# cafferychen777/flashdeconv

Measured on AMD Instinct MI355X. Metric: spots/sec to convergence (1M x 2000 x 30), higher is better.
Workload: dtype f64

## Files before the change

### flashdeconv_amd/_lib.py

```python
import ctypes
import os
import threading

import numpy as np

_HERE = os.path.dirname(os.path.abspath(__file__))
LIB_PATH = os.path.join(_HERE, "libfdx.so")

c_int = ctypes.c_int
c_i32 = ctypes.c_int32
c_i64 = ctypes.c_int64
c_double = ctypes.c_double
c_void_p = ctypes.c_void_p
c_size_t = ctypes.c_size_t
p_double = ctypes.POINTER(ctypes.c_double)
p_i64 = ctypes.POINTER(ctypes.c_int64)
p_i32 = ctypes.POINTER(ctypes.c_int32)


class FdxError(RuntimeError):
    """A libfdx call failed (message from fdx_last_error())."""


class SolveInfo(ctypes.Structure):
# ... 200 lines not shown
    "fdx_comm_init_loopback": (c_int, [c_i32, c_i32, ctypes.POINTER(c_void_p)]),
    "fdx_comm_destroy": (c_int, [c_void_p]),
    "fdx_comm_info": (c_int, [c_void_p, p_i32, p_i32]),
    "fdx_comm_rccl_count": (c_int, [c_void_p, p_i32]),
    "fdx_comm_allreduce_sum_dev": (c_int, [c_void_p, c_void_p, c_i32, c_void_p]),
    "fdx_sharded_solve_dev": (c_int, [c_void_p, c_void_p, c_void_p, c_i64, c_void_p, c_i32, c_double, c_double, c_double, c_i32,
                                      c_void_p, c_void_p, c_i64, ctypes.POINTER(SolveInfo), p_double, p_i32, c_void_p]),
    "fdx_solver_padded_k": (c_i32, [c_i32]),
    "fdx_shard_fit_dev": (c_int, [c_void_p, c_void_p, c_void_p, c_i32, c_i64, c_i32, c_i64, p_double, c_i32, p_i32, p_double, p_double,
                                  ctypes.POINTER(ShardFitParams), c_void_p, c_void_p, p_double, ctypes.POINTER(ShardFitInfo), c_void_p]),
    "fdx_sharded_solve_padded_dev": (c_int, [c_void_p, c_void_p, c_void_p, c_i64, c_void_p, c_i32, c_i32, c_double, c_double, c_double,
                                             c_i32, c_void_p, c_void_p, c_i64, ctypes.POINTER(SolveInfo), p_double, p_i32, c_void_p]),
    "fdx_tile_schedule": (c_int, [p_i32, p_double, c_i32, c_i32, c_i32, c_i32, c_i32, p_i32, p_i32, c_void_p, p_i32, p_double,
                                  c_void_p, c_i64]),
    "fdx_sketch_path": (c_int, [c_i32, c_void_p, c_i64, c_i32, c_i32, c_i32, c_i32, p_i32, p_double, p_i32, p_i32]),
    "fdx_column_sums": (c_int, [c_void_p, c_i32, c_i64, c_i32, p_double]),
    "fdx_log1p_f32": (c_int, [c_void_p, ctypes.c_float, c_i64, c_void_p]),
    "fdx_graph_build_knn": (c_int, [p_double, c_i64, c_i32, c_i32, ctypes.POINTER(c_void_p)]),
    "fdx_graph_build_radius": (c_int, [p_double, c_i64, c_i32, c_double, ctypes.POINTER(c_void_p)]),
    "fdx_nearest_distance": (c_int, [p_double, c_i64, c_i32, p_double]),
    "fdx_graph_export_csr": (c_int, [c_void_p, p_i64, p_i32]),
    "fdx_graph_from_csr": (c_int, [p_i64, p_i64, c_i64, ctypes.POINTER(c_void_p)]),
    "fdx_graph_destroy": (c_int, [c_void_p]),
    "fdx_graph_info": (c_int, [c_void_p, p_i64, p_i64, p_i32]),
    "fdx_graph_knn_ties": (c_int, [c_void_p, p_i64]),
    "fdx_graph_knn_far": (c_int, [c_void_p, ctypes.POINTER(c_i32)]),
    "fdx_kdtree_set_threads": (c_int, [c_i32]),
    "fdx_kdtree_tune": (c_int, [c_i32, c_i64]),
    "fdx_ckdtree_indices_dev": (c_int, [c_void_p, c_i64, c_i32, p_i64, p_i32, c_void_p]),
    "fdx_ckdtree_prebuild": (c_int, [p_double, c_void_p, c_i64, c_i32]),
# ... 135 lines not shown

def ptr_f64(a):
    return a.ctypes.data_as(p_double)


def ptr_i64(a):
    return a.ctypes.data_as(p_i64)


def ptr_i32(a):
    return a.ctypes.data_as(p_i32)


FDX_F32, FDX_F64 = 0, 1
PRE_RAW, PRE_LOG_CPM, PRE_LOG_CPM_SPARSE = 0, 1, 2
PRE_F64_MATH = 0x100


SRC_CODES = {"float32": 0, "float64": 1, "int8": 2, "uint8": 3, "bool": 3, "int16": 4, "uint16": 5, "int32": 6, "uint32": 7,
             "int64": 8, "uint64": 9}
_BIG = 32 << 20


def upload_bytes(dev_ptr, arr):
    if arr.nbytes >= _BIG and arr.nbytes % 4 == 0:
        check(load().fdx_upload_convert_dev(dev_ptr, FDX_F32, arr.ctypes.data_as(c_void_p), SRC_CODES["float32"], arr.nbytes // 4, None, None))
    elif arr.nbytes:
        check(load().fdx_memcpy_h2d(dev_ptr, arr.ctypes.data_as(c_void_p), arr.nbytes, None))


# ... 255 lines not shown
```

### flashdeconv_amd/csrc/fdx_kernels.h

```cpp
#pragma once
#include <cstdlib>
#include <hip/hip_runtime.h>

#include "../../include/fdx.h"
#include "spatial_sums.h"

#include <cstddef>
#include <cstdint>
#include <utility>
#include <initializer_list>

namespace fdx {

constexpr int FDX_MAX_K_FAST = 64;
constexpr int FDX_MAX_K_PAD = 96;
inline int solver_padded_K(int K) {
    if (K <= FDX_MAX_K_FAST || K > FDX_MAX_K_PAD) return K;
    for (int kp : {72, 80, 88, 96})
        if (K <= kp) return kp;
    return K;
}
inline bool sweep_instantiated(int K) { return K >= 1 && (K <= FDX_MAX_K_FAST || K == 72 || K == 80 || K == 88 || K == 96); }

struct BcdSweepArgs {
// ... 41 lines not shown
    const unsigned int* sched_pack = nullptr;
    unsigned long long end_mask = 0ULL;
    int pack_ok = 0;
    const double* gene_w = nullptr;
    const int* gene_bucket = nullptr;
    int scatter_ok = 0;
    const struct SketchPlan* owner = nullptr;
};
inline bool sketch_scatter_fits(int G, int d) {
    return d < 65535 && (((size_t)G + 256 + 7) & ~(size_t)7) * 10 + ((size_t)d + 64) * 8 <= 150 * 1024;
}
int launch_sketch_rows(const void* Y, int dtype, long long ldy, const int* row_map, long long n, int G, int d, int mode,
                       const SketchPlanDev& plan, double* Ys, long long ldys, double* row_sumsq, hipStream_t st);
bool fused_sketch_contract_ok(int dtype, long long ldy, const void* Y, int G, int d, int K, int mode, const SketchPlanDev& plan,
                              hipStream_t st = nullptr);
struct TileF64Math {
    bool prev;
    explicit TileF64Math(bool on);
    ~TileF64Math();
};
bool tile_sketch_ok(int dtype, long long ldy, const void* Y, int G, int d, int K, int mode, const SketchPlanDev& plan, hipStream_t st);
int launch_tile_sketch(const void* Y, int dtype, long long ldy, const int* row_map, long long n, int G, int d, int mode,
                       const SketchPlanDev& plan, const double* Xs, int K, double* H, long long ldh, double* row_sumsq,
                       hipStream_t st);
int launch_sketch_contract(const void* Y, int dtype, long long ldy, const int* row_map, long long n, int G, int d, int mode,
                           const SketchPlanDev& plan, const double* Xs, int K, double* H, long long ldh, double* row_sumsq,
                           hipStream_t st);
int column_sums_parts(long long n);
int launch_column_sums(const void* Y, int dtype, long long ldy, long long n, int G, double* partials, double* out,
                       hipStream_t st);
// ... 94 lines not shown
```

### flashdeconv_amd/csrc/fit.cpp

```cpp
#include "fdx_env.h"
#include <algorithm>
#include <cstdio>
#include <cmath>
#include <cstdlib>
#include <memory>
#include <vector>

#include "fdx_graph.h"
#include "fdx_internal.h"
#include "fdx_kernels.h"
#include "graph_build.h"
#include "prepare.h"
#include "sketch_plan.h"
#include "solver.h"
#include "x_cache.h"

using namespace fdx;

namespace {

int build_csc_from_tables(const int32_t* bucket, const double* weight, int G, int d, std::vector<long long>* col_ptr,
                          std::vector<int>* gene_idx, std::vector<double>* w) {
    col_ptr->assign((size_t)d + 1, 0);
    for (int g = 0; g < G; ++g) {
// ... 295 lines not shown
namespace {

std::unique_ptr<fdx_fit_carry> adopt_carry(const fdx_fit_params* prm) {
    return std::unique_ptr<fdx_fit_carry>(prm ? static_cast<fdx_fit_carry*>(prm->carry) : nullptr);
}

int fit_impl(const YSource& ysrc, int64_t n, int32_t G, const double* X, int32_t K, const int32_t* bucket,
             const double* weight_y, const double* weight_x, const double* coords_dev, int32_t dim,
             const fdx_fit_params* prm_in, std::unique_ptr<fdx_fit_carry> carry_in, fdx_graph** graph_inout, double* beta_out_dev,
             double* prop_out_dev, double* objectives_out, double* rel_changes_out, fdx_fit_info* info, void* stream) {
    FDX_REQUIRE(info != nullptr && prm_in != nullptr && graph_inout != nullptr, "fdx_fit_dev: null argument");
    fdx_fit_params prm_local = *prm_in;
    prm_local.mode_y &= 0xff;
    const fdx_fit_params* prm = &prm_local;
    TileF64Math f64_math((prm_in->mode_y & FDX_PRE_F64_MATH) != 0);
    std::memset(info, 0, sizeof(*info));
    const int32_t y_dtype = ysrc.row_dtype();
    FDX_REQUIRE(y_dtype == FDX_F32 || y_dtype == FDX_F64, "fdx_fit_dev: Y dtype must be FDX_F32 or FDX_F64");
    FDX_REQUIRE(n > 0 && G > 0 && K > 0, "fdx_fit_dev: empty problem");
    FDX_REQUIRE(n < 0x7fffff00LL, "fdx_fit_dev: n too large for one device");
    FDX_REQUIRE(ysrc.csr || ysrc.ldy >= G, "fdx_fit_dev: ldy < G");
    FDX_REQUIRE((ysrc.dense || ysrc.csr) && X && bucket && weight_y && weight_x, "fdx_fit_dev: null array");
    const int d = prm->sketch_dim;
    FDX_REQUIRE(d > 0, "fdx_fit_dev: sketch_dim must be positive");
    FDX_REQUIRE(prm->max_iter >= 0, "fdx_fit_dev: max_iter must be non-negative");
    hipStream_t st = (hipStream_t)stream;
    PoolStream pool_stream(st);
    Event t_begin(true), t_graph(true), eS0(true), eS1(true), t_solved(true), t_end(true);
    FDX_TRY(t_begin.record(st));
    trace_host("fit", "entry");
// ... 294 lines not shown
```

### flashdeconv_amd/csrc/prepare.cpp

```cpp
#include "prepare.h"

#include <algorithm>
#include <cstring>
#include <vector>

#include "fdx_env.h"
#include "fdx_kernels.h"
#include "solver.h"

namespace fdx {

int YTables::build(const YSource& y, int G, int d, int K, const int32_t* bucket, const double* weight_y, hipStream_t xs,
                   const char* who) {
    if (!y.csr) return sketch_plan_cached(bucket, weight_y, G, d, xs, &plan);
    csr_fused = csr_contract_ok(d, K, (y.csr->G + 31) / 32);
    return sel.build(y.gene_idx, G, y.csr->G, bucket, weight_y, d, csr_fused, xs, who);
}

namespace {
XCache<XSideBufs>& x_side_cache() {
    static XCache<XSideBufs>* const c = new XCache<XSideBufs>(4);
    return *c;
}
}
// ... 113 lines not shown
        Event sketched;
        FDX_TRY(sketched.record(st));
        FDX_TRY(sketched.wait_on(ys));
    }
    FDX_TRY(launch_sum_partials(row_sq, n, sum_dev, 1, 1, ys));
    if (yty_host) FDX_HIP(hipMemcpyAsync(yty_host, sum_dev, sizeof(double), hipMemcpyDeviceToHost, ys));
    if (done && ys != st) FDX_TRY(done->record(ys));
    return 0;
}

int prepare_queue(PrepareJob* job, const void* Y_dev, int y_dtype, long long n, int G, long long ldy, const int* row_map_dev,
                  const double* X, int K, const int* bucket, const double* weight_y, const double* weight_x, int d, int mode_y_in,
                  int mode_x, double* H_out_dev, long long ldh, double* XtX_host, hipStream_t st, const double* X_dev) {
    const int32_t mode_y = mode_y_in & 0xff;
    TileF64Math f64_math((mode_y_in & FDX_PRE_F64_MATH) != 0);
    FDX_REQUIRE(y_dtype == FDX_F32 || y_dtype == FDX_F64, "fdx_prepare_dev: Y dtype must be FDX_F32 or FDX_F64");
    FDX_REQUIRE(n >= 0 && G > 0 && K > 0 && d > 0, "fdx_prepare_dev: bad shape");
    FDX_REQUIRE(X && bucket && weight_y && weight_x && H_out_dev, "fdx_prepare_dev: null array");
    FDX_REQUIRE(ldh >= n && ldy >= G, "fdx_prepare_dev: leading dimension too small");
    YSource ysrc;
    ysrc.dense = Y_dev;
    ysrc.dtype = y_dtype;
    ysrc.ldy = ldy;
    hipStream_t side = fdx::env("FDX_NO_SIDE_STREAM") ? nullptr : library_side_stream();
    if (side == st) side = nullptr;
    job->side = side;
    const hipStream_t xs = side ? side : st;
    {
        PoolStream pool_xs(xs);
        FDX_TRY(job->y.build(ysrc, G, d, K, bucket, weight_y, xs, "fdx_prepare_dev"));
// ... 14 lines not shown
```

### flashdeconv_amd/csrc/tile_kernels.cpp

```cpp
#include "fdx_env.h"
#include <algorithm>
#include <cmath>
#include <cstdlib>
#include <memory>
#include <mutex>

#include "fdx_internal.h"
#include "fdx_kernels.h"
#include "sketch_plan.h"
#include "tile_device.h"
#include "tile_plan.h"
#include "tile_variant.h"

namespace fdx {

struct TilePlanDevice {
    TilePlanHost h;
    DevBuf w, off, len, ent_base, slot_bucket;
    int RS = 0;
    int WB = 0;
    size_t lds = 0;
};

const double* log_table_dev(hipStream_t st) {
    static std::mutex mu;
    static double* tabs[64] = {};
    int dev = 0;
    if (hipGetDevice(&dev) != hipSuccess || dev < 0 || dev >= 64) return nullptr;
    std::lock_guard<std::mutex> lock(mu);
    if (!tabs[dev]) {
        std::vector<double> t((size_t)LOG_TAB_N);
        for (int i = 0; i < LOG_TAB_N; ++i) {
            const unsigned bits = (unsigned)(LOG_TAB_BASE + i) << LOG_TAB_SHIFT;
            float c;
            std::memcpy(&c, &bits, 4);
            t[(size_t)i] = (double)(-logl((long double)c) + (long double)LOG_TAB_EXP_SHIFT * 0.693147180559945309417232121458176568L);
// ... 1 lines not shown
        double* p = nullptr;
        if (hipMalloc(&p, t.size() * sizeof(double)) != hipSuccess) return nullptr;
        if (hipMemcpyAsync(p, t.data(), t.size() * sizeof(double), hipMemcpyHostToDevice, st) != hipSuccess ||
            hipStreamSynchronize(st) != hipSuccess) {
            (void)hipFree(p);
            return nullptr;
        }
        tabs[dev] = p;
    }
    return tabs[dev];
}

static thread_local bool t_f64_math = false;
TileF64Math::TileF64Math(bool on) : prev(t_f64_math) { t_f64_math = on; }
TileF64Math::~TileF64Math() { t_f64_math = prev; }

static int tile_logv() {
    if (t_f64_math) return 0;
    const char* e = fdx::env("FDX_TILE_LOGV");
    return e ? atoi(e) : 2;
}

static bool tile_cfg(int dtype, int mode, int K, int d, int logv, TileVariant* out) {
    if ((dtype != FDX_F32 && dtype != FDX_F64) || K < 1 || K > 64 || d < 1) return false;
    if (mode != FDX_PRE_RAW && mode != FDX_PRE_LOG_CPM && mode != FDX_PRE_LOG_CPM_SPARSE) return false;
    const bool raw = mode == FDX_PRE_RAW;
    TileVariant v = raw ? TileVariant{12, 4, 11} : TileVariant{16, 0, 8};
    v.TT = (K + 15) / 16;
    if (K > 32 || d > 4 * v.NWC * v.JW) {
        v = raw ? TileVariant{12, 4, 22, 4, true} : TileVariant{8, 0, 32, 4, true};
// ... 62 lines not shown
        wg_tab.assign((size_t)t.h.NBLK * per, 0.0);
        for (int g = 0; g < sp.G; ++g)
            if (sp.host_bucket[(size_t)g] >= 0) wg_tab[(size_t)(g / t.h.GB) * per + g % t.h.GB] = sp.host_w[(size_t)g];
        for (size_t i = 0; i < t.h.off.size(); ++i)
            if (t.h.gene[i] < 0) t.h.off[i] = (unsigned short)t.h.GB;
    }
    if ((t.WB ? up(t.w, wg_tab.data(), wg_tab.size() * 8) : up(t.w, t.h.w.data(), t.h.w.size() * 8)) ||
        up(t.off, t.h.off.data(), t.h.off.size() * 2) || up(t.len, len_pad.data(), len_pad.size()) || up(t.ent_base, t.h.ent_base.data(), t.h.ent_base.size() * 4) ||
        up(t.slot_bucket, t.h.slot_bucket.data(), t.h.slot_bucket.size() * 4))
        return nullptr;
    if (hipStreamSynchronize(st) != hipSuccess) return nullptr;
    sp.tile[key] = std::move(best);
    return sp.tile[key].get();
}

__global__ void tile_xa_kernel(const double* __restrict__ Xs, const int* __restrict__ slot_bucket, int K, int d, int n_groups,
                               int TT, double* __restrict__ XA) {
    const int i = blockIdx.x * blockDim.x + threadIdx.x;
    if (i >= n_groups * TT * 64) return;
    const int lane = i & 63, t = (i >> 6) % TT, wj = (i >> 6) / TT;
    const int b = slot_bucket[wj * 4 + (lane >> 4)];
    const int type = t * 16 + (lane & 15);
    XA[i] = (b >= 0 && type < K) ? Xs[(size_t)type * d + b] : 0.0;
}

bool tile_sketch_ok(int dtype, long long ldy, const void* Y, int G, int d, int K, int mode, const SketchPlanDev& plan,
                    hipStream_t st) {
    if (!plan.owner) return false;
    TileVariant v;
    if (G <= 0 || !tile_cfg(dtype, mode, K, d, tile_logv(), &v)) return false;
    const int sz = dtype == FDX_F32 ? 4 : 8;
    if ((K > 32 || d > 512) && fdx::env("FDX_NO_TILE_WIDE")) return false;
    if (((size_t)G * sz) % 16 != 0 || ((size_t)ldy * sz) % 16 != 0 || (reinterpret_cast<uintptr_t>(Y) & 15) != 0) return false;
    return tile_plan_for(*plan.owner, dtype, mode, v, st) != nullptr;
}

int launch_tile_sketch(const void* Y, int dtype, long long ldy, const int* row_map, long long n, int G, int d, int mode,
                       const SketchPlanDev& plan, const double* Xs, int K, double* H, long long ldh, double* row_sumsq,
                       hipStream_t st) {
    if (n <= 0) return 0;
    TileVariant v;
    const TilePlanDevice* t = plan.owner && tile_cfg(dtype, mode, K, d, tile_logv(), &v) ? tile_plan_for(*plan.owner, dtype, mode, v, st) : nullptr;
    if (!t) return fail(FDX_ERR_INVALID, "tile sketch: no schedule for this shape");
    const void* kern = dtype == FDX_F32 ? tile_kernel<float>(mode, v) : tile_kernel<double>(mode, v);
    if (!kern) {
        char msg[128];
        std::snprintf(msg, sizeof msg, "tile sketch: no kernel for dtype %d mode %d, waves %d + %d x %d, TT %d, AVL2 %d, LOGV %d, WG %d",
                      dtype, mode, v.NWC, v.NWL, v.JW, v.TT, (int)v.avl2, v.logv, (int)v.wg);
        return fail(FDX_ERR_INVALID, msg);
    }
    TileArgs a{};
    a.ldy = ldy; a.n = n; a.ldh = ldh; a.G = G; a.d = d; a.K = K;
    a.NE = t->h.NE; a.GB = t->h.GB; a.NBLK = t->h.NBLK; a.RS = t->RS; a.jw_used = t->h.jw_used; a.WB = t->WB;
    const double* w_tab = t->w.as<double>();
    const unsigned short* off_tab = t->off.as<unsigned short>();
    const unsigned char* len_tab = t->len.as<unsigned char>();
    const int* ent_base = t->ent_base.as<int>();
    const int* slot_bucket = t->slot_bucket.as<int>();
// ... 73 lines not shown
    std::copy(h.slot_bucket.begin(), h.slot_bucket.end(), slot_bucket_out);
    std::copy(h.len.begin(), h.len.end(), len_out);
    std::copy(h.ent_base.begin(), h.ent_base.end(), ent_base_out);
    std::copy(h.w.begin(), h.w.end(), w_out);
    std::copy(h.off.begin(), h.off.end(), off_out);
    return 0;
}

extern "C" int fdx_sketch_path(int32_t y_dtype, const void* Y_dev, int64_t ldy, int32_t G, int32_t d, int32_t K, int32_t mode_y_in,
                               const int32_t* bucket, const double* weight_y, int32_t* path_out,
                               int32_t* dims_out ) {
    using namespace fdx;
    FDX_REQUIRE(bucket && weight_y && path_out, "fdx_sketch_path: null argument");
    FDX_REQUIRE(G > 0 && K > 0 && d > 0 && ldy >= G, "fdx_sketch_path: bad shape");
    const int32_t mode_y = mode_y_in & 0xff;
    if (dims_out) std::fill(dims_out, dims_out + 6, 0);
    hipStream_t st = nullptr;
    PoolStream pool_stream(st);
    std::shared_ptr<SketchPlan> plan;
    FDX_TRY(sketch_plan_cached(bucket, weight_y, G, d, st, &plan));
    *path_out = 0;
    if (!fused_sketch_contract_ok(y_dtype, ldy, Y_dev, G, d, K, mode_y, plan->dev(), st)) return 0;
    TileVariant v;
    const TilePlanDevice* t = tile_cfg(y_dtype, mode_y, K, d, tile_logv(), &v) ? tile_plan_for(*plan, y_dtype, mode_y, v, st) : nullptr;
    FDX_REQUIRE(t != nullptr, "fdx_sketch_path: the one-kernel form was accepted without a schedule");
    *path_out = v.wide ? 2 : 1;
    if (dims_out) {
        dims_out[0] = v.NWC; dims_out[1] = v.NWL; dims_out[2] = v.JW; dims_out[3] = v.TT;
        dims_out[4] = t->h.GB; dims_out[5] = t->h.NBLK;
    }
    return 0;
}
```

### flashdeconv_amd/csrc/tile_plan.cpp

```cpp
#include "tile_plan.h"

#include <algorithm>
#include <numeric>

namespace fdx {

bool build_tile_plan(const int* gene_bucket, const double* gene_w, int G, int d, int NW, int JW, int GB, TilePlanHost* out) {
    if (G <= 0 || d <= 0 || NW <= 0 || JW <= 0 || GB <= 0 || GB > 65536) return false;
    const int n_groups = NW * JW;
    if (d > 4 * n_groups) return false;
    const int NBLK = (G + GB - 1) / GB;
    TilePlanHost& p = *out;
    p = TilePlanHost();
    p.G = G; p.d = d; p.NW = NW; p.JW = JW; p.GB = GB; p.NBLK = NBLK;

    std::vector<std::vector<int>> genes((size_t)d);
    for (int g = 0; g < G; ++g) {
        const int b = gene_bucket[g];
        if (b < 0) continue;
        if (b >= d) return false;
        genes[(size_t)b].push_back(g);
    }
    std::vector<int> cnt((size_t)d * NBLK, 0);
    for (int b = 0; b < d; ++b)
// ... 95 lines not shown
            p.off.push_back(0);
            p.gene.push_back(-1);
        }
        p.steps += wave_steps;
        p.max_wave_steps = std::max(p.max_wave_steps, wave_steps);
        for (int j = 0; j < JW; ++j)
            for (int q = 0; q < 4; ++q) {
                const int b = groups[(size_t)of_wave[(size_t)w][(size_t)j]].b[q];
                if (b >= 0 && taken[(size_t)j * 4 + q] != (int)genes[(size_t)b].size()) return false;
            }
    }
    p.NE = (int)p.w.size();
    return true;
}

}
```

### flashdeconv_amd/csrc/tile_plan.h

```cpp
#pragma once
#include <vector>

namespace fdx {

struct TilePlanHost {
    int G = 0, d = 0, NW = 0, JW = 0, GB = 0, NBLK = 0;
    int NE = 0;
    int steps = 0;
    int max_wave_steps = 0;
    int jw_used = 0;
    std::vector<int> slot_bucket;
    std::vector<unsigned char> len;
    std::vector<int> ent_base;
    std::vector<double> w;
    std::vector<unsigned short> off;
    std::vector<int> gene;
};

bool build_tile_plan(const int* gene_bucket, const double* gene_w, int G, int d, int NW, int JW, int GB, TilePlanHost* out);


}
```

### flashdeconv_amd/csrc/tile_variant.h

```cpp
#pragma once
#include <cstddef>

namespace fdx {

constexpr int TILE_ROW_PAD = 16;

struct TileArgs {
    long long ldy, n, ldh;
    int G, d, K;
    int NE, GB, NBLK, RS, jw_used;
    int WB;
};

constexpr int JW_PAD(int jw) { return (jw + 7) & ~7; }

constexpr bool tile_red_pair(int NWC, bool AVL2) { return NWC > 8 || AVL2; }
constexpr int tile_red_th(int TT) { return TT > 2 ? 2 : TT; }
constexpr size_t tile_red_bytes(int NWC, bool AVL2, int TT) {
    return (size_t)(tile_red_pair(NWC, AVL2) ? NWC / 2 : NWC) * (tile_red_th(TT) * 4 * 64 + 64) * 8;
}

struct TileVariant {
    int NWC, NWL, JW, TT;
    bool wide, avl2;
    int logv;
    bool wg;
};

template <typename T> const void* tile_kernel(int mode, const TileVariant& v);

}
```

### include/fdx.h

```cpp
#ifndef FDX_H
#define FDX_H

#include <stddef.h>
#include <stdint.h>

#ifdef __cplusplus
extern "C" {
#endif

#define FDX_OK 0
#define FDX_ERR_INVALID (-1)
#define FDX_ERR_HIP (-2)
#define FDX_ERR_UNSUPPORTED (-3)
#define FDX_ERR_INTERNAL (-4)

#define FDX_F32 0
#define FDX_F64 1

#define FDX_PRE_RAW 0
#define FDX_PRE_LOG_CPM 1
#define FDX_PRE_LOG_CPM_SPARSE 2
#define FDX_PRE_F64_MATH 0x100

int fdx_version(void);
int fdx_env_reload(void);
const char* fdx_env_switch(int32_t i, const char** what_out);
const char* fdx_last_error(void);
int fdx_device_count(int* count);
int fdx_set_device(int device);
int fdx_device_name(char* buf, int buflen);

int fdx_malloc(void** dev_ptr, size_t bytes);
int fdx_free(void* dev_ptr);
int fdx_trim(void);
int fdx_x_cache_stats(int64_t out[4]);
int fdx_memcpy_h2d(void* dev_dst, const void* host_src, size_t bytes, void* stream);
int fdx_memcpy_d2h(void* host_dst, const void* dev_src, size_t bytes, void* stream);
// ... 10 lines not shown
#define FDX_SRC_U32 7
#define FDX_SRC_I64 8
#define FDX_SRC_U64 9
int fdx_upload_convert_dev(void* dst_dev, int32_t dst_dtype, const void* src_host, int32_t src_code, int64_t count,
                           double* max_abs_out, void* stream);
int fdx_download_dev(void* dst_host, const void* src_dev, size_t bytes, void* stream);
int fdx_pinned_copy_rate(size_t bytes, int32_t to_device, double* gbps_out);

int fdx_sketch(const void* Y, int32_t dtype, int64_t n, int32_t G, const int64_t* col_ptr, const int32_t* gene_idx,
               const double* weight, int32_t d, int32_t mode, double* Ys_out);
int fdx_tile_schedule(const int32_t* gene_bucket, const double* gene_w, int32_t G, int32_t d, int32_t NW, int32_t JW,
                      int32_t GB, int32_t* dims_out, int32_t* slot_bucket_out, uint8_t* len_out, int32_t* ent_base_out,
                      double* w_out, uint16_t* off_out, int64_t cap_entries);
int fdx_sketch_path(int32_t y_dtype, const void* Y_dev, int64_t ldy, int32_t G, int32_t d, int32_t K, int32_t mode_y,
                    const int32_t* bucket, const double* weight_y, int32_t* path_out, int32_t* dims_out);
int fdx_log1p_f32(const float* y, float scale, int64_t n, float* out);
int fdx_column_sums(const void* Y, int32_t dtype, int64_t n, int32_t G, double* sums_out);

int fdx_column_sums_dev(const void* Y_dev, int32_t dtype, int64_t n, int32_t G, int64_t ldy, double* sums_out_host,
                        void* stream);

int fdx_gene_moments_dev(const void* Y_dev, int32_t dtype, int64_t n, int32_t G, int64_t ldy, double* mean_out_host,
                         double* var_out_host, void* stream);
int fdx_gather_columns_dev(const void* Y_dev, int32_t dtype, int64_t n, int32_t G, int64_t ldy, const int32_t* idx_host,
                           int32_t G_sel, void* out_dev, void* stream);

int fdx_leverage_scores(const double* X, int32_t K, int32_t G, double regularization, double* lev_out);
typedef struct fdx_leverage_job fdx_leverage_job;
int fdx_leverage_begin(const double* X, int32_t K, int32_t G, double regularization, fdx_leverage_job** job);
int fdx_leverage_end(fdx_leverage_job* job, double* lev_out);
// ... 343 lines not shown
```

Baseline: 284.6 million.

## Add 64-spot tiled sketch kernel with per-wave gene batch schedule

Adds a new fused sketch-and-contract kernel that processes 64 spots per tile. Gene rows are double-buffered into LDS, per-wave batched gene schedules scatter weighted values into register accumulators, and the sketch is contracted against X with f64 MFMA after permlane swaps. A host-side planner builds the 64-spot batch schedule, and mode flags let callers force the 16- or 64-spot path. The aim is more reuse per loaded row and less scheduling overhead, at the cost of a much more complex kernel with high register pressure and possible occupancy limits.

```diff
diff --git a/flashdeconv_amd/_lib.py b/flashdeconv_amd/_lib.py
--- a/flashdeconv_amd/_lib.py
+++ b/flashdeconv_amd/_lib.py
@@ -238,6 +238,7 @@
     "fdx_tile_schedule": (c_int, [p_i32, p_double, c_i32, c_i32, c_i32, c_i32, c_i32, p_i32, p_i32, c_void_p, p_i32, p_double,
                                   c_void_p, c_i64]),
     "fdx_sketch_path": (c_int, [c_i32, c_void_p, c_i64, c_i32, c_i32, c_i32, c_i32, p_i32, p_double, p_i32, p_i32]),
+    "fdx_sketch_tile_spots": (c_int, [c_i32, c_void_p, c_i64, c_i32, c_i32, c_i32, c_i32, p_i32, p_double, c_i64, p_i32]),
     "fdx_column_sums": (c_int, [c_void_p, c_i32, c_i64, c_i32, p_double]),
     "fdx_log1p_f32": (c_int, [c_void_p, ctypes.c_float, c_i64, c_void_p]),
     "fdx_graph_build_knn": (c_int, [p_double, c_i64, c_i32, c_i32, ctypes.POINTER(c_void_p)]),
@@ -403,6 +404,7 @@
 
 FDX_F32, FDX_F64 = 0, 1
 PRE_RAW, PRE_LOG_CPM, PRE_LOG_CPM_SPARSE = 0, 1, 2
+PRE_TILE16, PRE_TILE64 = 0x200, 0x400
 PRE_F64_MATH = 0x100
 
 
diff --git a/flashdeconv_amd/csrc/fdx_kernels.h b/flashdeconv_amd/csrc/fdx_kernels.h
--- a/flashdeconv_amd/csrc/fdx_kernels.h
+++ b/flashdeconv_amd/csrc/fdx_kernels.h
@@ -79,6 +79,11 @@
                        const SketchPlanDev& plan, double* Ys, long long ldys, double* row_sumsq, hipStream_t st);
 bool fused_sketch_contract_ok(int dtype, long long ldy, const void* Y, int G, int d, int K, int mode, const SketchPlanDev& plan,
                               hipStream_t st = nullptr);
+struct TileSpotsForce {
+    int prev;
+    explicit TileSpotsForce(int mode_y_in);
+    ~TileSpotsForce();
+};
 struct TileF64Math {
     bool prev;
     explicit TileF64Math(bool on);
diff --git a/flashdeconv_amd/csrc/fit.cpp b/flashdeconv_amd/csrc/fit.cpp
--- a/flashdeconv_amd/csrc/fit.cpp
+++ b/flashdeconv_amd/csrc/fit.cpp
@@ -333,6 +333,7 @@
     prm_local.mode_y &= 0xff;
     const fdx_fit_params* prm = &prm_local;
     TileF64Math f64_math((prm_in->mode_y & FDX_PRE_F64_MATH) != 0);
+    TileSpotsForce tile_spots_force(prm_in->mode_y);
     std::memset(info, 0, sizeof(*info));
     const int32_t y_dtype = ysrc.row_dtype();
     FDX_REQUIRE(y_dtype == FDX_F32 || y_dtype == FDX_F64, "fdx_fit_dev: Y dtype must be FDX_F32 or FDX_F64");
diff --git a/flashdeconv_amd/csrc/hosttest/plan64_asan.cpp b/flashdeconv_amd/csrc/hosttest/plan64_asan.cpp
--- /dev/null
+++ b/flashdeconv_amd/csrc/hosttest/plan64_asan.cpp
@@ -0,0 +1,76 @@
+#include <cstdio>
+#include <cstring>
+#include <random>
+#include <vector>
+
+#include "../tile_plan.h"
+
+using namespace fdx;
+
+static int check_tile64(int G, int d, int GB16, int elem_bytes, unsigned seed) {
+    const int NW = T64_NW, JW = T64_JW, GB = T64_ROW_BYTES / elem_bytes;
+    std::mt19937 rng(seed);
+    std::vector<int> bucket((size_t)G);
+    std::vector<double> w((size_t)G);
+    for (int g = 0; g < G; ++g) {
+        bucket[(size_t)g] = (rng() % 41 == 0) ? -1 : (int)(rng() % (unsigned)d);
+        w[(size_t)g] = (rng() & 1) ? 1.0 + (rng() % 100) * 0.01 : -1.0 - (rng() % 100) * 0.01;
+    }
+    TilePlanHost p16;
+    if (!build_tile_plan(bucket.data(), w.data(), G, d, NW, JW, GB16, &p16)) return 1;
+    Tile64PlanHost p;
+    if (!build_tile64_plan(bucket.data(), w.data(), G, d, p16.slot_bucket.data(), NW, JW, GB, elem_bytes, &p)) return 2;
+    if (p.NBLK != (G + GB - 1) / GB || (int)p.words.size() != (p.n_batches + 2) * T64_BATCH_WORDS ||
+        (int)p.gene.size() != (p.n_batches + 2) * T64_U || (int)p.batch_base.size() != NW * (3 * p.NBLK + 1))
+        return 3;
+    std::vector<int> seen((size_t)G, 0), last((size_t)d, -1);
+    int at = 0;
+    for (int wv = 0; wv < NW; ++wv) {
+        const int* bb = p.batch_base.data() + (size_t)wv * (3 * p.NBLK + 1);
+        if (bb[0] != at) return 4;
+        for (int c = 0; c < p.NBLK; ++c)
+            for (int seg = 0; seg < 3; ++seg)
+                for (int b = bb[3 * c + seg]; b < bb[3 * c + seg + 1]; ++b, ++at) {
+                    if (b != at) return 5;
+                    const int* e = p.words.data() + (size_t)b * T64_BATCH_WORDS;
+                    for (int u = 0; u < T64_U; ++u) {
+                        const unsigned m = (unsigned)e[2 * T64_U + u];
+                        const int idx = (int)((m >> 16) & 0xff), off = (int)(m & 0xffffu);
+                        double wt;
+                        const unsigned long long bits = ((unsigned long long)(unsigned)e[2 * u + 1] << 32) | (unsigned)e[2 * u];
+                        std::memcpy(&wt, &bits, 8);
+                        if ((int)(m >> 24) != seg || idx >= 16 || seg * 16 + idx >= JW * 4 || off + elem_bytes > T64_ROW_BYTES) return 6;
+                        const int g = p.gene[(size_t)b * T64_U + u];
+                        if (g < 0) {
+                            if (wt != 0.0 || off != 0) return 7;
+                            continue;
+                        }
+                        const int own = p16.slot_bucket[(size_t)wv * JW * 4 + seg * 16 + idx];
+                        if (g / GB != c || own != bucket[(size_t)g] || wt != w[(size_t)g] || off != (g % GB) * elem_bytes) return 8;
+                        if (g <= last[(size_t)own]) return 9;
+                        last[(size_t)own] = g;
+                        ++seen[(size_t)g];
+                    }
+                }
+        if (bb[3 * p.NBLK] != at) return 10;
+    }
+    if (at != p.n_batches) return 11;
+    for (int g = 0; g < G; ++g)
+        if (seen[(size_t)g] != (bucket[(size_t)g] >= 0 ? 1 : 0)) return 12;
+    for (size_t i = (size_t)p.n_batches * T64_U; i < p.gene.size(); ++i)
+        if (p.gene[i] != -1) return 13;
+    return 0;
+}
+
+int main() {
+    int bad = 0;
+    const int shapes[][4] = {{2000, 512, 1024, 4}, {2000, 528, 1024, 4}, {1500, 256, 384, 8}, {600, 64, 768, 4}, {64, 512, 256, 4},
+                             {256, 64, 256, 4}, {4, 8, 256, 4}, {2, 1, 128, 8}};
+    for (const auto& s : shapes)
+        for (unsigned seed = 1; seed <= 3; ++seed) {
+            const int rc = check_tile64(s[0], s[1], s[2], s[3], seed);
+            if (rc) { std::printf("tile64 plan G=%d d=%d GB16=%d bytes=%d seed=%u: error %d\n", s[0], s[1], s[2], s[3], seed, rc); ++bad; }
+        }
+    std::printf(bad ? "FAILED\n" : "64-spot schedule builder: ok under the sanitizers\n");
+    return bad ? 1 : 0;
+}
diff --git a/flashdeconv_amd/csrc/prepare.cpp b/flashdeconv_amd/csrc/prepare.cpp
--- a/flashdeconv_amd/csrc/prepare.cpp
+++ b/flashdeconv_amd/csrc/prepare.cpp
@@ -151,6 +151,7 @@
                   int mode_x, double* H_out_dev, long long ldh, double* XtX_host, hipStream_t st, const double* X_dev) {
     const int32_t mode_y = mode_y_in & 0xff;
     TileF64Math f64_math((mode_y_in & FDX_PRE_F64_MATH) != 0);
+    TileSpotsForce tile_spots_force(mode_y_in);
     FDX_REQUIRE(y_dtype == FDX_F32 || y_dtype == FDX_F64, "fdx_prepare_dev: Y dtype must be FDX_F32 or FDX_F64");
     FDX_REQUIRE(n >= 0 && G > 0 && K > 0 && d > 0, "fdx_prepare_dev: bad shape");
     FDX_REQUIRE(X && bucket && weight_y && weight_x && H_out_dev, "fdx_prepare_dev: null array");
diff --git a/flashdeconv_amd/csrc/tile64_inst.cpp b/flashdeconv_amd/csrc/tile64_inst.cpp
--- /dev/null
+++ b/flashdeconv_amd/csrc/tile64_inst.cpp
@@ -0,0 +1,17 @@
+#include "tile64_sketch_kernel.h"
+
+#ifndef FDX_TILE_F64
+#error "compile with -DFDX_TILE_F64=<0|1>"
+#endif
+
+namespace fdx {
+
+using TileT = std::conditional<FDX_TILE_F64, double, float>::type;
+
+template <> const void* tile64_kernel<TileT>(int TT) {
+    if (TT == 1) return (const void*)tile64_sketch_kernel<TileT, 1>;
+    if (TT == 2) return (const void*)tile64_sketch_kernel<TileT, 2>;
+    return nullptr;
+}
+
+}
diff --git a/flashdeconv_amd/csrc/tile64_sketch_kernel.h b/flashdeconv_amd/csrc/tile64_sketch_kernel.h
--- /dev/null
+++ b/flashdeconv_amd/csrc/tile64_sketch_kernel.h
@@ -0,0 +1,229 @@
+#pragma once
+#include <type_traits>
+
+#include "tile_sketch_kernel.h"
+
+namespace fdx {
+
+typedef double t64_d16 __attribute__((ext_vector_type(16)));
+
+template <int I0, int I1, typename F> __device__ __forceinline__ void t64_static_for(F&& f) {
+    if constexpr (I0 < I1) {
+        f(std::integral_constant<int, I0>{});
+        t64_static_for<I0 + 1, I1>(f);
+    }
+}
+
+__device__ __forceinline__ void t64_swap32(double& a, double& b) {
+    const auto lo = __builtin_amdgcn_permlane32_swap((unsigned)__double2loint(a), (unsigned)__double2loint(b), false, false);
+    const auto hi = __builtin_amdgcn_permlane32_swap((unsigned)__double2hiint(a), (unsigned)__double2hiint(b), false, false);
+    a = __hiloint2double((int)hi[0], (int)lo[0]);
+    b = __hiloint2double((int)hi[1], (int)lo[1]);
+}
+__device__ __forceinline__ void t64_swap16(double& a, double& b) {
+    const auto lo = __builtin_amdgcn_permlane16_swap((unsigned)__double2loint(a), (unsigned)__double2loint(b), false, false);
+    const auto hi = __builtin_amdgcn_permlane16_swap((unsigned)__double2hiint(a), (unsigned)__double2hiint(b), false, false);
+    a = __hiloint2double((int)hi[0], (int)lo[0]);
+    b = __hiloint2double((int)hi[1], (int)lo[1]);
+}
+
+template <typename T, int TT>
+__global__ __launch_bounds__(T64_NW * 64, T64_NW / 4) void tile64_sketch_kernel(
+    const TileArgs a, const T* __restrict__ Yp, const int* __restrict__ row_map, const double* __restrict__ Xs,
+    double* __restrict__ H, double* __restrict__ row_sumsq, const int* __restrict__ ent, const int* __restrict__ batch_base,
+    const int* __restrict__ slot_bucket) {
+    extern __shared__ __attribute__((aligned(16))) unsigned char smem[];
+    static_assert(TT == 1 || TT == 2, "narrow form: one or two type tiles");
+    constexpr int NW = T64_NW, JW = T64_JW, U = T64_U, W = T64_BATCH_WORDS;
+    constexpr int RPL = (T64_ROWS + NW - 1) / NW;
+    constexpr int NR = NW / 2;
+    constexpr int TS = 4 * 64;
+    static_assert(tile64_red_bytes() == (size_t)2 * NR * (TS + 64) * 8, "the reduction area overlays a stage buffer");
+    const int tid = threadIdx.x, lane = tid & 63;
+    const int wave = __builtin_amdgcn_readfirstlane(tid >> 6);
+    const int r = lane & 15, q = lane >> 4;
+    const int stage_bytes = T64_ROWS * a.RS;
+    const long long n_tiles = (a.n + T64_ROWS - 1) / T64_ROWS;
+    long long tile = blockIdx.x;
+    if (tile >= n_tiles) return;
+
+    auto load_rows = [&](long long t, const T* (&rp)[RPL]) {
+#pragma unroll
+        for (int k = 0; k < RPL; ++k) {
+            const int rr = wave + NW * k;
+            rp[k] = nullptr;
+            if (rr >= T64_ROWS || t >= n_tiles) continue;
+            const long long sp = t * T64_ROWS + rr;
+            if (sp < a.n) {
+                const long long row = row_map ? (long long)row_map[sp] : sp;
+                rp[k] = Yp + (size_t)row * (size_t)a.ldy;
+            }
+        }
+    };
+    auto issue_stage = [&](const T* const (&rp)[RPL], int c, int buf) {
+        const int gene0 = c * a.GB;
+        const int bytes = (min(a.GB, a.G - gene0)) * (int)sizeof(T);
+        unsigned char* base = smem + (size_t)buf * stage_bytes;
+#pragma unroll
+        for (int k = 0; k < RPL; ++k) {
+            if (!rp[k]) continue;
+            const unsigned char* src = reinterpret_cast<const unsigned char*>(rp[k] + gene0) + lane * 16;
+            if (lane * 16 < bytes) dma16(src, base + (wave + NW * k) * a.RS);
+        }
+    };
+    const T* rowp[RPL];
+    const T* rown[RPL];
+    load_rows(tile, rowp);
+    issue_stage(rowp, 0, 0);
+
+    const int* bb = batch_base + wave * (3 * a.NBLK + 1);
+    int buf = 0;
+    for (; tile < n_tiles; tile += gridDim.x) {
+        const bool has_next = tile + gridDim.x < n_tiles;
+        load_rows(tile + gridDim.x, rown);
+        t64_d16 A = (t64_d16)(0.0), B = (t64_d16)(0.0);
+        t64_d16 C = (t64_d16)(0.0);
+        for (int c = 0; c < a.NBLK; ++c) {
+            __builtin_amdgcn_s_waitcnt(0x0f70);
+            lds_barrier();
+            if (c + 1 < a.NBLK) issue_stage(rowp, c + 1, buf ^ 1);
+            else if (has_next) issue_stage(rown, 0, buf ^ 1);
+            const unsigned rowb = (unsigned)buf * (unsigned)stage_bytes + (unsigned)lane * (unsigned)a.RS;
+            int b = bb[3 * c];
+            const int b1 = bb[3 * c + 1], b2 = bb[3 * c + 2], b3 = bb[3 * c + 3];
+            auto fetch = [&](int (&e)[W], int bi) {
+#pragma unroll
+                for (int i = 0; i < W; ++i) e[i] = ent[(size_t)bi * W + i];
+            };
+            auto read = [&](T (&y)[U], const int (&e)[W]) {
+#pragma unroll
+                for (int u = 0; u < U; ++u) y[u] = *reinterpret_cast<const T*>(smem + rowb + ((unsigned)e[2 * U + u] & 0xffffu));
+            };
+            int e[W], en[W];
+            T y[U];
+            fetch(e, b);
+            fetch(en, b + 1);
+            read(y, e);
+            auto run = [&](auto& V, int bend) __attribute__((always_inline)) {
+                while (b < bend) {
+                    double yd[U];
+#pragma unroll
+                    for (int u = 0; u < U; ++u) yd[u] = (double)y[u];
+                    __builtin_amdgcn_sched_barrier(0);
+                    read(y, en);
+                    int e2[W];
+                    fetch(e2, b + 2);
+                    __builtin_amdgcn_sched_barrier(0);
+#pragma unroll
+                    for (int u = 0; u < U; ++u) {
+                        const int i = (e[2 * U + u] >> 16) & 15;
+                        V[i] = fma(__hiloint2double(e[2 * u + 1], e[2 * u]), yd[u], V[i]);
+                    }
+                    ++b;
+#pragma unroll
+                    for (int i = 0; i < W; ++i) {
+                        e[i] = en[i];
+                        en[i] = e2[i];
+                    }
+                }
+            };
+            run(A, b1);
+            run(B, b2);
+            run(C, b3);
+            buf ^= 1;
+        }
+#pragma unroll
+        for (int k = 0; k < RPL; ++k) rowp[k] = rown[k];
+
+        double av[JW];
+        auto load_av = [&](int t) {
+            int sb0 = wave * JW * 4;
+            asm volatile("" : "+s"(sb0));
+#pragma unroll
+            for (int j = 0; j < JW; ++j) {
+                const int c0 = slot_bucket[sb0 + j * 4], c1 = slot_bucket[sb0 + j * 4 + 1], c2 = slot_bucket[sb0 + j * 4 + 2],
+                          c3 = slot_bucket[sb0 + j * 4 + 3];
+                const int b = q == 0 ? c0 : q == 1 ? c1 : q == 2 ? c2 : c3;
+                const int type = t * 16 + r;
+                const bool ok = b >= 0 && type < a.K;
+                const double v = Xs[(size_t)(ok ? type : 0) * a.d + (ok ? b : 0)];
+                av[j] = ok ? v : 0.0;
+            }
+        };
+        load_av(0);
+        auto get = [&](auto jc, auto qc) -> double {
+            constexpr int J = decltype(jc)::value, QQ = decltype(qc)::value;
+            if constexpr (J < 4) return A[J * 4 + QQ];
+            else if constexpr (J < 8) return B[(J - 4) * 4 + QQ];
+            else return C[(J - 8) * 4 + QQ];
+        };
+        auto set = [&](auto jc, auto qc, double v) {
+            constexpr int J = decltype(jc)::value, QQ = decltype(qc)::value;
+            if constexpr (J < 4) A[J * 4 + QQ] = v;
+            else if constexpr (J < 8) B[(J - 4) * 4 + QQ] = v;
+            else C[(J - 8) * 4 + QQ] = v;
+        };
+        using I0 = std::integral_constant<int, 0>;
+        using I1 = std::integral_constant<int, 1>;
+        using I2 = std::integral_constant<int, 2>;
+        using I3 = std::integral_constant<int, 3>;
+        t64_static_for<0, JW>([&](auto jc) {
+            double r0 = get(jc, I0{}), r1 = get(jc, I1{}), r2 = get(jc, I2{}), r3 = get(jc, I3{});
+            t64_swap32(r0, r2);
+            t64_swap32(r1, r3);
+            t64_swap16(r0, r1);
+            t64_swap16(r2, r3);
+            set(jc, I0{}, r0);
+            set(jc, I1{}, r1);
+            set(jc, I2{}, r2);
+            set(jc, I3{}, r3);
+        });
+        double* red_base = reinterpret_cast<double*>(smem + (size_t)(buf ^ 1) * stage_bytes);
+        lds_barrier();
+        t64_static_for<0, 4 * TT>([&](auto rc) {
+            constexpr int TI = decltype(rc)::value / 4, S = decltype(rc)::value % 4;
+            if (TI > 0 && S == 0) load_av(TI);
+            using SC = std::integral_constant<int, S>;
+            double* red = red_base + (size_t)(decltype(rc)::value & 1) * NR * (TS + 64);
+            double* red_sq = red + (size_t)NR * TS;
+            double4_t accm = double4_t{0.0, 0.0, 0.0, 0.0};
+            double sq = 0.0;
+            t64_static_for<0, JW>([&](auto jc) {
+                constexpr int J = decltype(jc)::value;
+                const double bv = get(jc, SC{});
+                accm = __builtin_amdgcn_mfma_f64_16x16x4f64(av[J], bv, accm, 0, 0, 0);
+                if (TI == 0) sq = fma(bv, bv, sq);
+            });
+            if (wave >= NR) {
+#pragma unroll
+                for (int rr = 0; rr < 4; ++rr) red[(size_t)(wave - NR) * TS + rr * 64 + lane] = accm[rr];
+                if (TI == 0) red_sq[(wave - NR) * 64 + lane] = sq;
+            }
+            lds_barrier();
+            if (wave < NR) {
+#pragma unroll
+                for (int rr = 0; rr < 4; ++rr) red[(size_t)wave * TS + rr * 64 + lane] += accm[rr];
+                if (TI == 0) red_sq[wave * 64 + lane] += sq;
+            }
+            lds_barrier();
+            const long long s0 = tile * T64_ROWS + S * TILE_ROWS;
+            if (tid < TS) {
+                double sum = 0.0;
+#pragma unroll
+                for (int v = 0; v < NR; ++v) sum += red[(size_t)v * TS + tid];
+                const int type = TI * 16 + (lane >> 4) + 4 * (tid >> 6);
+                const long long sp = s0 + (lane & 15);
+                if (type < a.K && sp < a.n) H[(size_t)type * a.ldh + sp] = sum;
+            }
+            if (TI == 0 && row_sumsq && tid < TILE_ROWS && s0 + tid < a.n) {
+                double sum = 0.0;
+                for (int v = 0; v < NR; ++v)
+#pragma unroll
+                    for (int qq = 0; qq < 4; ++qq) sum += red_sq[v * 64 + qq * 16 + tid];
+                row_sumsq[s0 + tid] = sum;
+            }
+        });
+    }
+}
+
+}
diff --git a/flashdeconv_amd/csrc/tile_kernels.cpp b/flashdeconv_amd/csrc/tile_kernels.cpp
--- a/flashdeconv_amd/csrc/tile_kernels.cpp
+++ b/flashdeconv_amd/csrc/tile_kernels.cpp
@@ -14,12 +14,19 @@
 
 namespace fdx {
 
+struct Tile64PlanDevice {
+    Tile64PlanHost h;
+    DevBuf words, batch_base;
+};
+
 struct TilePlanDevice {
     TilePlanHost h;
     DevBuf w, off, len, ent_base, slot_bucket;
     int RS = 0;
     int WB = 0;
     size_t lds = 0;
+    mutable std::unique_ptr<Tile64PlanDevice> t64;
+    mutable bool t64_tried = false;
 };
 
 const double* log_table_dev(hipStream_t st) {
@@ -51,6 +58,12 @@
 static thread_local bool t_f64_math = false;
 TileF64Math::TileF64Math(bool on) : prev(t_f64_math) { t_f64_math = on; }
 TileF64Math::~TileF64Math() { t_f64_math = prev; }
+
+static thread_local int t_tile_spots = 0;
+TileSpotsForce::TileSpotsForce(int mode_y_in) : prev(t_tile_spots) {
+    t_tile_spots = (mode_y_in & FDX_PRE_TILE64) ? 64 : (mode_y_in & FDX_PRE_TILE16) ? 16 : 0;
+}
+TileSpotsForce::~TileSpotsForce() { t_tile_spots = prev; }
 
 static int tile_logv() {
     if (t_f64_math) return 0;
@@ -143,6 +156,55 @@
     return sp.tile[key].get();
 }
 
+static int tile_spots(int mode, const TileVariant& v) {
+    const bool can = mode == FDX_PRE_RAW && !v.wide && v.NWC == T64_NW && v.JW == T64_JW;
+    return can && t_tile_spots == 64 ? 64 : 16;
+}
+
+static const Tile64PlanDevice* tile64_plan_for(const SketchPlan& sp, int dtype, const TilePlanDevice& t, hipStream_t st) {
+    std::lock_guard<std::mutex> lock(sp.tile_mu);
+    if (t.t64_tried) return t.t64.get();
+    t.t64_tried = true;
+    const int sz = dtype == FDX_F32 ? 4 : 8;
+    auto p = std::make_unique<Tile64PlanDevice>();
+    if (!build_tile64_plan(sp.host_bucket.data(), sp.host_w.data(), sp.G, sp.d, t.h.slot_bucket.data(), T64_NW, T64_JW,
+                           T64_ROW_BYTES / sz, sz, &p->h))
+        return nullptr;
+    if (p->words.alloc(p->h.words.size() * 4) || copy_h2d(p->words.p, p->h.words.data(), p->h.words.size() * 4, st) ||
+        p->batch_base.alloc(p->h.batch_base.size() * 4) ||
+        copy_h2d(p->batch_base.p, p->h.batch_base.data(), p->h.batch_base.size() * 4, st))
+        return nullptr;
+    if (hipStreamSynchronize(st) != hipSuccess) return nullptr;
+    if (fdx::env("FDX_DEBUG"))
+        std::fprintf(stderr, "[fdx] tile64 plan: G=%d d=%d GB=%d blocks=%d batches=%d (%d entries for %d genes)\n", sp.G, sp.d, p->h.GB,
+                     p->h.NBLK, p->h.n_batches, p->h.n_batches * T64_U, sp.G);
+    t.t64 = std::move(p);
+    return t.t64.get();
+}
+
+static int launch_tile64(const void* Y, int dtype, long long ldy, const int* row_map, long long n, int G, int d, const SketchPlan& sp,
+                         const TilePlanDevice& t, const TileVariant& v, const double* Xs, int K, double* H, long long ldh,
+                         double* row_sumsq, hipStream_t st) {
+    const Tile64PlanDevice* p = tile64_plan_for(sp, dtype, t, st);
+    if (!p) return fail(FDX_ERR_INVALID, "tile sketch: no 64-spot schedule for this shape");
+    const void* kern = dtype == FDX_F32 ? tile64_kernel<float>(v.TT) : tile64_kernel<double>(v.TT);
+    if (!kern) return fail(FDX_ERR_INVALID, "tile sketch: no 64-spot kernel for this number of type tiles");
+    TileArgs a{};
+    a.ldy = ldy; a.n = n; a.ldh = ldh; a.G = G; a.d = d; a.K = K;
+    a.GB = p->h.GB; a.NBLK = p->h.NBLK; a.RS = T64_ROW_BYTES + TILE_ROW_PAD;
+    const int* ent = p->words.as<int>();
+    const int* batch_base = p->batch_base.as<int>();
+    const int* slot_bucket = t.slot_bucket.as<int>();
+    const long long n_tiles = (n + T64_ROWS - 1) / T64_ROWS;
+    const int grid = (int)std::min<long long>(n_tiles, 256);
+    const size_t lds = tile64_lds_bytes();
+    FDX_HIP(hipFuncSetAttribute(kern, hipFuncAttributeMaxDynamicSharedMemorySize, (int)lds));
+    void* args[] = {(void*)&a, (void*)&Y, (void*)&row_map, (void*)&Xs, (void*)&H, (void*)&row_sumsq, (void*)&ent, (void*)&batch_base,
+                    (void*)&slot_bucket};
+    FDX_HIP(hipLaunchKernel(kern, dim3(grid), dim3(T64_NW * 64), args, lds, st));
+    return 0;
+}
+
 __global__ void tile_xa_kernel(const double* __restrict__ Xs, const int* __restrict__ slot_bucket, int K, int d, int n_groups,
                                int TT, double* __restrict__ XA) {
     const int i = blockIdx.x * blockDim.x + threadIdx.x;
@@ -171,6 +233,7 @@
     TileVariant v;
     const TilePlanDevice* t = plan.owner && tile_cfg(dtype, mode, K, d, tile_logv(), &v) ? tile_plan_for(*plan.owner, dtype, mode, v, st) : nullptr;
     if (!t) return fail(FDX_ERR_INVALID, "tile sketch: no schedule for this shape");
+    if (tile_spots(mode, v) == 64) return launch_tile64(Y, dtype, ldy, row_map, n, G, d, *plan.owner, *t, v, Xs, K, H, ldh, row_sumsq, st);
     const void* kern = dtype == FDX_F32 ? tile_kernel<float>(mode, v) : tile_kernel<double>(mode, v);
     if (!kern) {
         char msg[128];
@@ -274,6 +337,7 @@
     FDX_REQUIRE(bucket && weight_y && path_out, "fdx_sketch_path: null argument");
     FDX_REQUIRE(G > 0 && K > 0 && d > 0 && ldy >= G, "fdx_sketch_path: bad shape");
     const int32_t mode_y = mode_y_in & 0xff;
+    TileSpotsForce tile_spots_force(mode_y_in);
     if (dims_out) std::fill(dims_out, dims_out + 6, 0);
     hipStream_t st = nullptr;
     PoolStream pool_stream(st);
@@ -288,6 +352,25 @@
     if (dims_out) {
         dims_out[0] = v.NWC; dims_out[1] = v.NWL; dims_out[2] = v.JW; dims_out[3] = v.TT;
         dims_out[4] = t->h.GB; dims_out[5] = t->h.NBLK;
-    }
-    return 0;
-}
+        if (tile_spots(mode_y, v) == 64) {
+            const Tile64PlanDevice* p = tile64_plan_for(*plan, y_dtype, *t, st);
+            FDX_REQUIRE(p != nullptr, "fdx_sketch_path: no 64-spot schedule for a shape that qualifies");
+            dims_out[1] = 0; dims_out[4] = p->h.GB; dims_out[5] = p->h.NBLK;
+        }
+    }
+    return 0;
+}
+
+extern "C" int fdx_sketch_tile_spots(int32_t y_dtype, const void* Y_dev, int64_t ldy, int32_t G, int32_t d, int32_t K, int32_t mode_y_in,
+                                     const int32_t* bucket, const double* weight_y, int64_t n, int32_t* spots_out) {
+    using namespace fdx;
+    FDX_REQUIRE(spots_out != nullptr && n >= 0, "fdx_sketch_tile_spots: bad argument");
+    TileSpotsForce tile_spots_force(mode_y_in);
+    int32_t path = 0;
+    FDX_TRY(fdx_sketch_path(y_dtype, Y_dev, ldy, G, d, K, mode_y_in, bucket, weight_y, &path, nullptr));
+    *spots_out = 0;
+    TileVariant v;
+    if (path == 0 || !tile_cfg(y_dtype, mode_y_in & 0xff, K, d, tile_logv(), &v)) return 0;
+    *spots_out = tile_spots(mode_y_in & 0xff, v);
+    return 0;
+}
diff --git a/flashdeconv_amd/csrc/tile_plan.cpp b/flashdeconv_amd/csrc/tile_plan.cpp
--- a/flashdeconv_amd/csrc/tile_plan.cpp
+++ b/flashdeconv_amd/csrc/tile_plan.cpp
@@ -1,6 +1,7 @@
 #include "tile_plan.h"
 
 #include <algorithm>
+#include <cstring>
 #include <numeric>
 
 namespace fdx {
@@ -133,4 +134,68 @@
     return true;
 }
 
+bool build_tile64_plan(const int* gene_bucket, const double* gene_w, int G, int d, const int* slot_bucket, int NW, int JW,
+                       int GB, int elem_bytes, Tile64PlanHost* out) {
+    if (G <= 0 || d <= 0 || NW <= 0 || JW <= 0 || GB <= 0 || (elem_bytes != 4 && elem_bytes != 8)) return false;
+    if ((long long)GB * elem_bytes > 65536 || JW * 4 > 3 * 16) return false;
+    std::vector<int> owner((size_t)d, -1);
+    for (int i = 0; i < NW * JW * 4; ++i) {
+        const int b = slot_bucket[i];
+        if (b < 0) continue;
+        if (b >= d || owner[(size_t)b] >= 0) return false;
+        owner[(size_t)b] = i;
+    }
+    Tile64PlanHost& p = *out;
+    p = Tile64PlanHost();
+    p.GB = GB;
+    p.NBLK = (G + GB - 1) / GB;
+    const int NSEG = 3;
+    std::vector<std::vector<int>> lists((size_t)NW * p.NBLK * NSEG);
+    for (int g = 0; g < G; ++g) {
+        const int b = gene_bucket[g];
+        if (b < 0) continue;
+        if (b >= d || owner[(size_t)b] < 0) return false;
+        const int w = owner[(size_t)b] / (JW * 4), s = owner[(size_t)b] % (JW * 4);
+        lists[((size_t)w * p.NBLK + g / GB) * NSEG + s / 16].push_back(g);
+    }
+    auto put_batch = [&](const int* genes, int cnt, int seg) {
+        const size_t at = p.words.size();
+        p.words.resize(at + T64_BATCH_WORDS, 0);
+        int fill = 0;
+        if (cnt > 0) fill = (owner[(size_t)gene_bucket[genes[0]]] % (JW * 4)) % 16;
+        for (int u = 0; u < T64_U; ++u) {
+            double wt = 0.0;
+            int idx = fill, off = 0, gid = -1;
+            if (u < cnt) {
+                gid = genes[u];
+                wt = gene_w[gid];
+                idx = (owner[(size_t)gene_bucket[gid]] % (JW * 4)) % 16;
+                off = (gid % GB) * elem_bytes;
+            }
+            unsigned long long bits;
+            static_assert(sizeof bits == sizeof wt, "64-bit doubles");
+            std::memcpy(&bits, &wt, 8);
+            p.words[at + 2 * u] = (int)(unsigned)(bits & 0xffffffffULL);
+            p.words[at + 2 * u + 1] = (int)(unsigned)(bits >> 32);
+            p.words[at + 2 * T64_U + u] = (int)(((unsigned)seg << 24) | ((unsigned)idx << 16) | (unsigned)off);
+            p.gene.push_back(gid);
+        }
+    };
+    const int per_wave = NSEG * p.NBLK + 1;
+    p.batch_base.assign((size_t)NW * per_wave, 0);
+    for (int w = 0; w < NW; ++w) {
+        for (int c = 0; c < p.NBLK; ++c)
+            for (int seg = 0; seg < NSEG; ++seg) {
+                p.batch_base[(size_t)w * per_wave + c * NSEG + seg] = (int)(p.words.size() / T64_BATCH_WORDS);
+                const std::vector<int>& L = lists[((size_t)w * p.NBLK + c) * NSEG + seg];
+                for (size_t i = 0; i < L.size(); i += T64_U) put_batch(L.data() + i, (int)std::min<size_t>(T64_U, L.size() - i), seg);
+            }
+        p.batch_base[(size_t)w * per_wave + NSEG * p.NBLK] = (int)(p.words.size() / T64_BATCH_WORDS);
+    }
+    p.n_batches = (int)(p.words.size() / T64_BATCH_WORDS);
+    put_batch(nullptr, 0, 0);
+    put_batch(nullptr, 0, 0);
+    return true;
 }
+
+}
diff --git a/flashdeconv_amd/csrc/tile_plan.h b/flashdeconv_amd/csrc/tile_plan.h
--- a/flashdeconv_amd/csrc/tile_plan.h
+++ b/flashdeconv_amd/csrc/tile_plan.h
@@ -1,5 +1,7 @@
 #pragma once
 #include <vector>
+
+#include "tile_variant.h"
 
 namespace fdx {
 
@@ -19,5 +21,14 @@
 
 bool build_tile_plan(const int* gene_bucket, const double* gene_w, int G, int d, int NW, int JW, int GB, TilePlanHost* out);
 
+struct Tile64PlanHost {
+    int GB = 0, NBLK = 0, n_batches = 0;
+    std::vector<int> batch_base;
+    std::vector<int> words;
+    std::vector<int> gene;
+};
+bool build_tile64_plan(const int* gene_bucket, const double* gene_w, int G, int d, const int* slot_bucket, int NW, int JW,
+                       int GB, int elem_bytes, Tile64PlanHost* out);
+
 
 }
diff --git a/flashdeconv_amd/csrc/tile_variant.h b/flashdeconv_amd/csrc/tile_variant.h
--- a/flashdeconv_amd/csrc/tile_variant.h
+++ b/flashdeconv_amd/csrc/tile_variant.h
@@ -29,4 +29,13 @@
 
 template <typename T> const void* tile_kernel(int mode, const TileVariant& v);
 
+constexpr int T64_ROWS = 64, T64_NW = 12, T64_JW = 11;
+constexpr int T64_ROW_BYTES = 1024;
+constexpr int T64_U = 4;
+constexpr int T64_BATCH_WORDS = 3 * T64_U;
+constexpr size_t tile64_red_bytes() { return (size_t)2 * (T64_NW / 2) * (4 * 64 + 64) * 8; }
+constexpr size_t tile64_lds_bytes() { return (size_t)2 * T64_ROWS * (T64_ROW_BYTES + TILE_ROW_PAD); }
+static_assert(tile64_red_bytes() <= tile64_lds_bytes() / 2, "the reduction areas fit a stage buffer");
+template <typename T> const void* tile64_kernel(int TT);
+
 }
diff --git a/include/fdx.h b/include/fdx.h
--- a/include/fdx.h
+++ b/include/fdx.h
@@ -21,6 +21,8 @@
 #define FDX_PRE_LOG_CPM 1
 #define FDX_PRE_LOG_CPM_SPARSE 2
 #define FDX_PRE_F64_MATH 0x100
+#define FDX_PRE_TILE16 0x200
+#define FDX_PRE_TILE64 0x400
 
 int fdx_version(void);
 int fdx_env_reload(void);
@@ -61,6 +63,8 @@
                       double* w_out, uint16_t* off_out, int64_t cap_entries);
 int fdx_sketch_path(int32_t y_dtype, const void* Y_dev, int64_t ldy, int32_t G, int32_t d, int32_t K, int32_t mode_y,
                     const int32_t* bucket, const double* weight_y, int32_t* path_out, int32_t* dims_out);
+int fdx_sketch_tile_spots(int32_t y_dtype, const void* Y_dev, int64_t ldy, int32_t G, int32_t d, int32_t K, int32_t mode_y,
+                          const int32_t* bucket, const double* weight_y, int64_t n, int32_t* spots_out);
 int fdx_log1p_f32(const float* y, float scale, int64_t n, float* out);
 int fdx_column_sums(const void* Y, int32_t dtype, int64_t n, int32_t G, double* sums_out);
 
```

New measurement: 274.8 million. -3.4%, worse.
